# nianticlabs/wavelet-monodepth

Measured on AMD Instinct MI355X. Metric: decoder+IDWT frames/sec @640x192 bs12, higher is better.
Workload: dtype f32; 1 GPU; KITTI ResNet18 640x192 dense wavelet decoder + 4x Haar IDWT, forward, batch 12 per GPU (BASELINE.json configs[1]); encoder features resident in HBM; batch_per_gpu=12, global_batch=12, parallelism=dp1 (independent shards)

## Files before the change

wavelet_monodepth_amd/csrc/wmd_conv_fwd.hip:

```cpp
#include <algorithm>
#include <cstdlib>
#include <cstring>
#include <type_traits>
#include "wmd_conv_common.h"

namespace wmd {

template <int TH, int TW, int MR, int NR, int WM, int WN, int CK, int TAPS, int NBUF = 2>
struct ConvTile {
    static constexpr int NT = WM * WN * 64;
    static constexpr int HALO = (TAPS == 9) ? 1 : 0;
    static constexpr int PH = TH + 2 * HALO;
    static constexpr int PW = TW + 2 * HALO;
    static constexpr int NPOSITIONS = PH * PW;
    static constexpr int PS = ((NPOSITIONS - 16 + 31) / 32) * 32 + 16;
    static constexpr int NPOS = (NPOSITIONS + NT - 1) / NT;
    static constexpr int NPIX = TH * TW;
    static constexpr int A_RUN = (CK / 4) * TAPS * 64;
    static constexpr int A_FLOATS = WM * MR * A_RUN;
    static constexpr int B_FLOATS = CK * PS;
    static constexpr int NAV = (A_FLOATS / 4 + NT - 1) / NT;
    static constexpr int LDS_FLOATS = NBUF * (B_FLOATS + A_FLOATS);
    static_assert(WN * NR * 16 >= NPIX, "tile has more pixels than MFMA columns");
    static_assert(CK % 4 == 0, "CK must be a whole number of 4-channel K-steps");
    static_assert(A_FLOATS % 4 == 0, "the weight tile is moved in 16-byte pieces (a partial last wave is exec-masked)");
    static_assert(TW % 4 == 0, "four consecutive pixels of an accumulator row must not straddle image rows");
};

template <int TH, int TW, int MR, int NR, int WM, int WN, int CK, int TAPS, bool FUSE = false, int NBUF = 2>
__global__ __launch_bounds__(WM* WN * 64) void conv_fwd_kernel(const ConvKArgs a) {
    using T = ConvTile<TH, TW, MR, NR, WM, WN, CK, TAPS, NBUF>;
    constexpr int NT = T::NT, HALO = T::HALO, PW = T::PW, PS = T::PS, NPOS = T::NPOS;
    constexpr int KSTEPS = CK / 4;

    constexpr int MID_FLOATS = FUSE ? WM * MR * 16 * T::PS : 0;
    __shared__ __attribute__((aligned(16))) float lds[T::LDS_FLOATS > MID_FLOATS ? T::LDS_FLOATS : MID_FLOATS];
    float* ldsA = lds + NBUF * T::B_FLOATS;
    const int tid = threadIdx.x;
    const int lane = tid & 63;
    const int wave = __builtin_amdgcn_readfirstlane(tid >> 6);
    const int wm = wave % WM;
    const int wn = wave / WM;

    int t, by;
    if (a.cob > 0) {
        const int item = xcd_contiguous(blockIdx.x, gridDim.x);
        t = item / a.cob;
        by = item - t * a.cob;
    } else {
        t = xcd_contiguous(blockIdx.x, gridDim.x);
        by = blockIdx.y;
    }
    const int tx = t % a.tiles_x;
    t /= a.tiles_x;
    const int ty = t % a.tiles_y;
    const int b = t / a.tiles_y;
    const int y0 = ty * TH, x0 = tx * TW;
    const int ks = blockIdx.z;
    const int H = a.H, W = a.W;

    constexpr unsigned kOOB = 0x80000000u;
    unsigned ob1[NPOS], ob2[NPOS];
#pragma unroll
    for (int i = 0; i < NPOS; ++i) {
        const int p = tid + i * NT;
        const int py = p / PW, px = p % PW;
        int gy = y0 + py - HALO, gx = x0 + px - HALO;
        bool ok = p < T::NPOSITIONS;
        if (HALO) {
            ok = pad_coord(gy, H, a.pad_mode) && ok;
            ok = pad_coord(gx, W, a.pad_mode) && ok;
        }
        ok = ok && gy < H && gx < W && gy >= 0 && gx >= 0;
        gy = min(max(gy, 0), H - 1);
        gx = min(max(gx, 0), W - 1);
        ob2[i] = ok ? (unsigned)(gy * W + gx) * 4u : kOOB;
        int sy = gy - a.shift1, sx = gx - a.shift1;
        if (a.up1 == 2) {
            sy = gy >> 1;
            sx = gx >> 1;
        }
        const bool ok1 = ok && sy >= 0 && sx >= 0 && sy < a.H1 && sx < a.W1;
        ob1[i] = ok1 ? (unsigned)(sy * a.W1 + sx) * 4u : kOOB;
    }

    const size_t plane1 = (size_t)a.H1 * a.W1, plane2 = (size_t)H * W;
    const float* x1b = a.x1 + (size_t)b * a.C1 * plane1;
// ... 80 lines not shown
#pragma unroll
            for (int m = 0; m < MR; ++m) wf[slot][m] = asrc[m * T::A_RUN + (kk * TAPS + tp) * 64];
#pragma unroll
            for (int n = 0; n < NR; ++n) pf[slot][n] = bsrc[boff[n] + kk * 4 * PS + ky * PW + kx];
        };
#pragma unroll
        for (int s = 0; s < D && s < S; ++s) fetch(s);
#pragma unroll
        for (int s = 0; s < S; ++s) {
            if constexpr (PREFETCH) {
#pragma unroll
                for (int q = 0; q < NPIECES; ++q)
                    if (q * SP / NPIECES == s) stage_piece(c + 1, buf ^ 1, q);
            }
            if (s + D < S) fetch(s + D);
            __builtin_amdgcn_sched_barrier(0);
#pragma unroll
            for (int m = 0; m < MR; ++m)
#pragma unroll
                for (int n = 0; n < NR; ++n)
                    acc[m][n] = __builtin_amdgcn_mfma_f32_16x16x4f32(pf[s % RS][n], wf[s % RS][m], acc[m][n], 0, 0, 0);
            __builtin_amdgcn_sched_barrier(0);
        }
        __syncthreads();
    };
    if constexpr (NBUF == 2) {
        for (int c = c_begin; c + 1 < c_end; ++c) chunk_body(c, std::true_type{});
        if (c_begin < c_end) chunk_body(c_end - 1, std::false_type{});
    } else {
        for (int c = c_begin; c < c_end; ++c) chunk_body(c, std::false_type{});
    }

    if constexpr (FUSE) {
        static_assert(!FUSE || TAPS == 1, "the fused head is a 1x1 chain");
        constexpr int CO_T = WM * MR * 16, PS2 = T::PS, R2W = WM >= 2 ? 1 : 2;
        float* mid = lds;
#pragma unroll
        for (int m = 0; m < MR; ++m) {
            const int chl = (wm * MR + m) * 16 + (lane & 15);
            const float bv = bias_v[m];
#pragma unroll
            for (int n = 0; n < NR; ++n) {
                const int q = (wn * NR + n) * 16 + (lane >> 4) * 4;
                float4 v;
                v.x = act_apply(acc[m][n][0] + bv, a.act, a.slope);
                v.y = act_apply(acc[m][n][1] + bv, a.act, a.slope);
                v.z = act_apply(acc[m][n][2] + bv, a.act, a.slope);
                v.w = act_apply(acc[m][n][3] + bv, a.act, a.slope);
                *reinterpret_cast<float4*>(mid + chl * PS2 + q) = v;
            }
        }
        __syncthreads();
        if (WM > 2 && wm >= 2) return;
        f32x4 acc2[R2W][NR];
#pragma unroll
        for (int j = 0; j < R2W; ++j)
#pragma unroll
            for (int n = 0; n < NR; ++n) acc2[j][n] = f32x4{0.f, 0.f, 0.f, 0.f};
        constexpr int NCI4_2 = CO_T / 4;
        const float* w2 = a.wp2 + (size_t)by * (2 * NCI4_2 * 64) + lane;
        const float* msrc = mid + (lane >> 4) * PS2 + (lane & 15);
        constexpr int QD = NCI4_2 < 8 ? NCI4_2 : 8;
        float wq[QD][R2W];
#pragma unroll
        for (int q = 0; q < QD; ++q)
#pragma unroll
            for (int j = 0; j < R2W; ++j) wq[q][j] = w2[((WM == 1 ? j : wm) * NCI4_2 + q) * 64];
#pragma unroll
        for (int k4 = 0; k4 < NCI4_2; ++k4) {
            float pf[NR], wf[R2W];
#pragma unroll
            for (int j = 0; j < R2W; ++j) wf[j] = wq[k4 % QD][j];
            if (k4 + QD < NCI4_2) {
#pragma unroll
                for (int j = 0; j < R2W; ++j) wq[k4 % QD][j] = w2[((WM == 1 ? j : wm) * NCI4_2 + k4 + QD) * 64];
            }
#pragma unroll
            for (int n = 0; n < NR; ++n) pf[n] = msrc[k4 * 4 * PS2 + (wn * NR + n) * 16];
#pragma unroll
            for (int j = 0; j < R2W; ++j)
#pragma unroll
                for (int n = 0; n < NR; ++n) acc2[j][n] = __builtin_amdgcn_mfma_f32_16x16x4f32(pf[n], wf[j], acc2[j][n], 0, 0, 0);
        }
        const bool vec = (W & 3) == 0;
#pragma unroll
        for (int j = 0; j < R2W; ++j) {
            const int r2 = (WM == 1 ? j : wm) * 16 + (lane & 15);
            if (r2 >= 27) continue;
            float* tb = a.t + ((size_t)b * a.t_ctot + a.t_row0 + by * 27 + r2) * plane2;
#pragma unroll
            for (int n = 0; n < NR; ++n) {
                const int ox = x0 + (wn * NR + n) * 16 + (lane >> 4) * 4;
                if (ox >= W) continue;
                if (vec && ox + 3 < W) {
                    *reinterpret_cast<float4*>(tb + ox) = make_float4(acc2[j][n][0], acc2[j][n][1], acc2[j][n][2], acc2[j][n][3]);
                } else {
#pragma unroll
                    for (int r = 0; r < 4; ++r)
                        if (ox + r < W) tb[ox + r] = acc2[j][n][r];
                }
            }
        }
        return;
    }

    const bool final_out = (a.ksplit == 1);
    float* ybase = a.y + ((size_t)ks * a.B + b) * a.Cout * plane2;
    const bool vec_ok = (W & 3) == 0;
#pragma unroll
    for (int m = 0; m < MR; ++m) {
        const int co = ((by * WM + wm) * MR + m) * 16 + (lane & 15);
        const float bv = final_out ? bias_v[m] : 0.f;
#pragma unroll
        for (int n = 0; n < NR; ++n) {
            const int q = (wn * NR + n) * 16 + (lane >> 4) * 4;
            const int oy = y0 + q / TW, ox = x0 + q % TW;
            if (co >= a.Cout || q >= T::NPIX || oy >= H || ox >= W) continue;
            float v[4];
#pragma unroll
            for (int r = 0; r < 4; ++r) {
                v[r] = acc[m][n][r];
                if (final_out) v[r] = act_apply(v[r] + bv, a.act, a.slope);
            }
            float* dst = ybase + (size_t)co * plane2 + (size_t)oy * W + ox;
            if (final_out && a.gate) {
                const float* gp = a.gate + ((size_t)b * a.Cout + co) * plane2 + (size_t)oy * W + ox;
                if (vec_ok && ox + 3 < W) {
                    const float4 gv = *reinterpret_cast<const float4*>(gp);
                    v[0] *= act_deriv(gv.x, a.gate_act, a.gate_slope);
                    v[1] *= act_deriv(gv.y, a.gate_act, a.gate_slope);
                    v[2] *= act_deriv(gv.z, a.gate_act, a.gate_slope);
                    v[3] *= act_deriv(gv.w, a.gate_act, a.gate_slope);
                } else {
#pragma unroll
                    for (int r = 0; r < 4; ++r)
                        if (ox + r < W) v[r] *= act_deriv(gp[r], a.gate_act, a.gate_slope);
                }
            }
            if (vec_ok && ox + 3 < W) {
                *reinterpret_cast<float4*>(dst) = make_float4(v[0], v[1], v[2], v[3]);
            } else {
#pragma unroll
                for (int r = 0; r < 4; ++r)
                    if (ox + r < W) dst[r] = v[r];
            }
        }
    }
}

__global__ void conv_splitk_reduce_kernel(const float* __restrict__ partial, const float* __restrict__ bias,
                                          float* __restrict__ y, size_t n, size_t plane, int Cout, int ksplit,
                                          int act, float slope, const float* __restrict__ gate, int gate_act, float gate_slope,
                                          const uint8_t* __restrict__ out_mask) {
    for (size_t i = (size_t)blockIdx.x * blockDim.x + threadIdx.x; i < n; i += (size_t)gridDim.x * blockDim.x) {
        float v = 0.f;
        int s = 0;
        if (out_mask && out_mask[i / (plane * Cout) * plane + i % plane] == 0) {
            y[i] = 0.f;
            continue;
        }
        for (; s + 4 <= ksplit; s += 4) {
            const float p0 = partial[(size_t)s * n + i], p1 = partial[(size_t)(s + 1) * n + i];
            const float p2 = partial[(size_t)(s + 2) * n + i], p3 = partial[(size_t)(s + 3) * n + i];
            v = (((v + p0) + p1) + p2) + p3;
        }
        for (; s < ksplit; ++s) v += partial[(size_t)s * n + i];
        if (bias) v += bias[(i / plane) % Cout];
        v = act_apply(v, act, slope);
        if (gate) v *= act_deriv(gate[i], gate_act, gate_slope);
        y[i] = v;
    }
}

constexpr int kRedCh = 8;
__global__ __launch_bounds__(256) void conv_splitk_reduce_list_kernel(const float* __restrict__ partial, const float* __restrict__ bias,
                                                                      float* __restrict__ y, const int* __restrict__ tile_list,
                                                                      const int* __restrict__ tile_count, const uint8_t* __restrict__ out_mask,
                                                                      int B, int Cout, int H, int W, int TH, int TW, int tiles_x, int tiles_y,
                                                                      int cob, int nchunks, int ksmax, int slots, int act, float slope) {
    const int n_act = list_total(tile_count, B);
    if ((int)blockIdx.x >= n_act) return;
    int ks, cps;
    list_ksplit(n_act * cob, nchunks, ksmax, slots, ks, cps);
// ... 1075 lines not shown
```

wavelet_monodepth_amd/csrc/wmd_head.hip:

```cpp
#include <algorithm>
#include <cstdlib>
#include "wmd_internal.h"
#include "wmd_head_shiftsum.h"

namespace wmd {



constexpr int HT_H = 16, HT_W = 32, H_CK = 8, H_TT = 128;
constexpr int H_PH = HT_H + 2;
constexpr int H_PWV = HT_W + 2;
constexpr int H_PW = 36;
constexpr int H_PS = H_PH * H_PW + 4;

template <int COUT>
struct HeadSmem {
    float patch[2][H_CK * H_PS];
    float wgt[2][H_CK * COUT * 12];
    float dump[64];
};

template <int COUT, int NG>
__device__ __forceinline__ void head_side(const float* __restrict__ x, size_t bstride, const float* __restrict__ wgt,
                                          int C, int c_begin, int c_end, int H, int W, int b, int y0, int x0,
// ... 188 lines not shown
                sp[q] = 1.f / (1.f + expf(-accp[co][q]));
                if (a.mode == 1) {
                    r[q] = a.scale * sp[q];
                } else {
                    sn[q] = 1.f / (1.f + expf(-accn[co][q]));
                    r[q] = a.scale * sp[q] - a.scale * sn[q];
                }
            }
        }
        float* yo = a.y + o + co * plane;
        if (vec) {
            *reinterpret_cast<float4*>(yo) = make_float4(r[0], r[1], r[2], r[3]);
            if (a.mode >= 1 && a.sig_p) *reinterpret_cast<float4*>(a.sig_p + o + co * plane) = make_float4(sp[0], sp[1], sp[2], sp[3]);
            if (a.mode == 2 && a.sig_n) *reinterpret_cast<float4*>(a.sig_n + o + co * plane) = make_float4(sn[0], sn[1], sn[2], sn[3]);
        } else {
#pragma unroll
            for (int q = 0; q < 4; ++q)
                if (ox + q < a.W) {
                    yo[q] = r[q];
                    if (a.mode >= 1 && a.sig_p) a.sig_p[o + co * plane + q] = sp[q];
                    if (a.mode == 2 && a.sig_n) a.sig_n[o + co * plane + q] = sn[q];
                }
        }
    }
}

__global__ void head_finalize_kernel(const wmd_head_args a, const float* __restrict__ partial, int csplit) {
    const size_t plane = (size_t)a.H * a.W;
    const size_t n = (size_t)a.B * a.Cout * plane;
    for (size_t i = (size_t)blockIdx.x * blockDim.x + threadIdx.x; i < n; i += (size_t)gridDim.x * blockDim.x) {
        const size_t pix = i % plane;
        const int co = (i / plane) % a.Cout;
        const int b = i / (plane * a.Cout);
        float p = a.bias_p ? a.bias_p[co] : 0.f, q = (a.mode == 2 && a.bias_n) ? a.bias_n[co] : 0.f;
        for (int cs = 0; cs < csplit; ++cs) {
            const float* pp = partial + (((size_t)cs * a.B + b) * 2 * a.Cout) * plane + pix;
            p += pp[(size_t)co * plane];
            if (a.mode == 2) q += pp[(size_t)(a.Cout + co) * plane];
        }
        float r;
        if (a.mode == 0) {
            r = a.scale * p;
        } else {
            const float sp = 1.f / (1.f + expf(-p));
            if (a.sig_p) a.sig_p[i] = sp;
            if (a.mode == 1) {
                r = a.scale * sp;
            } else {
                const float sn = 1.f / (1.f + expf(-q));
                if (a.sig_n) a.sig_n[i] = sn;
                r = a.scale * sp - a.scale * sn;
            }
        }
        a.y[i] = r;
    }
}

__global__ void head_shiftsum_kernel(const wmd_head_shiftsum_args a) {
    const int H = a.H, W = a.W;
    const size_t plane = (size_t)H * W;
    const size_t total = (size_t)a.B * plane;
    const size_t total_w = (total + 63) / 64 * 64;
    for (size_t i0 = (size_t)blockIdx.x * blockDim.x + threadIdx.x; i0 < total_w; i0 += (size_t)gridDim.x * blockDim.x) {
        const bool live = i0 < total;
        const size_t i = live ? i0 : total - 1;
        const int x = i % W;
        const int y = (i / W) % H;
        const size_t b = i / plane;
        int off[9];
        float okf[9];
#pragma unroll
        for (int t = 0; t < 9; ++t) {
            int gy = y + t / 3 - 1, gx = x + t % 3 - 1;
            const bool ok = pad_coord(gy, H, a.pad_mode) & pad_coord(gx, W, a.pad_mode);
            gy = min(max(gy, 0), H - 1);
            gx = min(max(gx, 0), W - 1);
            off[t] = gy * W + gx;
            okf[t] = ok ? 1.f : 0.f;
        }
        const float* tb = a.t + b * (a.yl_out ? 81 : 54) * plane;
        const bool in_mask = !a.yh_mask || a.yh_mask[b * plane + (size_t)y * W + x] != 0;
        const bool wave_any = __builtin_amdgcn_ballot_w64(in_mask && live) != 0;
        float yh[3] = {0.f, 0.f, 0.f};
        if (wave_any) {
            float vp[27], vn[27];
#pragma unroll
            for (int k = 0; k < 27; ++k) {
                vp[k] = tb[(size_t)k * plane + off[k % 9]];
                vn[k] = tb[(size_t)(27 + k) * plane + off[k % 9]];
            }
#pragma unroll
            for (int co = 0; co < 3; ++co) {
                float sp = a.bias_p ? a.bias_p[co] : 0.f, sn = a.bias_n ? a.bias_n[co] : 0.f;
#pragma unroll
                for (int t = 0; t < 9; ++t) {
                    sp += okf[t] * vp[co * 9 + t];
                    sn += okf[t] * vn[co * 9 + t];
                }
                const float a1 = fast_sigmoid(sp), a2 = fast_sigmoid(sn);
                yh[co] = in_mask ? a.scale * a1 - a.scale * a2 : 0.f;
                if (a.sig_p && live) {
                    a.sig_p[(b * 3 + co) * plane + (size_t)y * W + x] = a1;
                    a.sig_n[(b * 3 + co) * plane + (size_t)y * W + x] = a2;
                }
            }
        }
        if (live) {
#pragma unroll
            for (int co = 0; co < 3; ++co) a.yh[(b * 3 + co) * plane + (size_t)y * W + x] = yh[co];
        }
        float l = 0.f;
        if (a.yl_out) {
            float sl = a.bias_ll ? a.bias_ll[0] : 0.f;
#pragma unroll
            for (int t = 0; t < 9; ++t) sl += okf[t] * tb[(size_t)(54 + t) * plane + off[t]];
            const float sgl = fast_sigmoid(sl);
            l = a.scale_ll * sgl;
            if (live) a.yl_out[i] = l;
            if (live && a.sig_ll) a.sig_ll[i] = sgl;
        } else if (a.yl) {
            l = a.yl[i];
        }
        if ((a.yl || a.yl_out) && a.out) {
            float v[4] = {(l + yh[0] + yh[1] + yh[2]) * 0.5f, (l + yh[0] - yh[1] - yh[2]) * 0.5f,
                          (l - yh[0] + yh[1] - yh[2]) * 0.5f, (l - yh[0] - yh[1] + yh[2]) * 0.5f};
            if (a.range_keys) {
                float lo = live ? fminf(fminf(v[0], v[1]), fminf(v[2], v[3])) : INFINITY;
                float hi = live ? fmaxf(fmaxf(v[0], v[1]), fmaxf(v[2], v[3])) : -INFINITY;
                const int b0 = __builtin_amdgcn_readfirstlane((int)b);
                const bool uniform = __builtin_amdgcn_ballot_w64((int)b != b0) == 0;
                if (uniform) {
#pragma unroll
                    for (int o = 32; o > 0; o >>= 1) {
                        lo = fminf(lo, __shfl_xor(lo, o));
                        hi = fmaxf(hi, __shfl_xor(hi, o));
                    }
                }
                if ((uniform ? (threadIdx.x & 63) == 0 : live) && lo <= hi) {
                    const unsigned ul = __float_as_uint(lo), uh = __float_as_uint(hi);
                    atomicMin(&a.range_keys[2 * b], (ul & 0x80000000u) ? ~ul : (ul | 0x80000000u));
                    atomicMax(&a.range_keys[2 * b + 1], (uh & 0x80000000u) ? ~uh : (uh | 0x80000000u));
                }
            }
            if (!live) continue;
            const size_t dst = b * 4 * plane + (size_t)(2 * y) * (2 * W) + 2 * x;
            *reinterpret_cast<float2*>(a.out + dst) = make_float2(v[0], v[1]);
            *reinterpret_cast<float2*>(a.out + dst + 2 * W) = make_float2(v[2], v[3]);
            if (a.disp) {
#pragma unroll
                for (int k = 0; k < 4; ++k) {
                    v[k] *= a.disp_scale;
                    if (a.clamp01) v[k] = fminf(fmaxf(v[k], 0.f), 1.f);
                }
                *reinterpret_cast<float2*>(a.disp + dst) = make_float2(v[0], v[1]);
                *reinterpret_cast<float2*>(a.disp + dst + 2 * W) = make_float2(v[2], v[3]);
            }
        }
    }
}

struct ShiftsumChainArgs {
    wmd_head_shiftsum_args lv[3];
    int n;
    int by0, bx0;
};


__global__ __launch_bounds__(256) void head_shiftsum_chain_kernel(const ShiftsumChainArgs c) {
    __shared__ float low[2][256];
    const int by0 = c.by0, bx0 = c.bx0;
    const int H0 = c.lv[0].H, W0 = c.lv[0].W;
    const int tiles_x = (W0 + bx0 - 1) / bx0, tiles_y = (H0 + by0 - 1) / by0;
    int t = blockIdx.x;
    const int tx = t % tiles_x;
    t /= tiles_x;
    const int ty = t % tiles_y;
    const size_t b = t / tiles_y;
    const int tid = threadIdx.x;
    for (int k = 0; k < c.n; ++k) {
        const int sy = by0 << k, sx = bx0 << k;
        if (tid < sy * sx) {
            const int py = tid / sx, px = tid % sx;
            const int y = ty * sy + py, x = tx * sx + px;
            if (y < c.lv[k].H && x < c.lv[k].W) {
                float v[4];
                shiftsum_pixel(c.lv[k], b, y, x, k > 0, k > 0 ? low[(k - 1) & 1][py * sx + px] : 0.f, v);
                if (k + 1 < c.n) {
                    float* nl = low[k & 1];
                    const int ns = sx * 2;
                    nl[(2 * py) * ns + 2 * px] = v[0];
                    nl[(2 * py) * ns + 2 * px + 1] = v[1];
                    nl[(2 * py + 1) * ns + 2 * px] = v[2];
                    nl[(2 * py + 1) * ns + 2 * px + 1] = v[3];
                }
            }
        }
        __syncthreads();
    }
// ... 122 lines not shown
```

wavelet_monodepth_amd/csrc/wmd_head_chain.hip:

```cpp
#include <algorithm>
#include <cstdlib>
#include <type_traits>
#include <utility>
#include "wmd_internal.h"

#ifndef WMD_CHAIN_PD256
#define WMD_CHAIN_PD256 4
#endif
#ifndef WMD_CHAIN_PD128
#define WMD_CHAIN_PD128 1
#endif

namespace wmd {

typedef float f32x4 __attribute__((ext_vector_type(4)));

template <class F, int... I>
__device__ __forceinline__ void hc_static_for_impl(F&& f, std::integer_sequence<int, I...>) {
    (f(std::integral_constant<int, I>{}), ...);
}
template <int N, class F>
__device__ __forceinline__ void hc_static_for(F&& f) {
    hc_static_for_impl(f, std::make_integer_sequence<int, N>{});
}

__device__ __forceinline__ void hc_barrier() {
    asm volatile("s_waitcnt lgkmcnt(0)" ::: "memory");
    __builtin_amdgcn_s_barrier();
    asm volatile("" ::: "memory");
}

struct HeadChainArgs {
    const float* x;
    const float* wp1;
    const float* bias1;
    const float* wp2;
    float* t;
    int plane, tiles, t_planes;
    int C;
    float slope;
    const uint8_t* run_mask;
    const float* ll_wp1;
    const float* ll_bias1;
    const float* ll_wp2;
    float* mid_out;
    int mid_ct, mid_off[3];
};

template <int C, int RS, int PG, int NT, int KC>
struct HeadChainTile {
    static constexpr int NW = RS * PG, NTH = NW * 64;
    static constexpr int PXB = PG * NT * 16;
    static constexpr int MTS = C / 16;
    static constexpr int MT = MTS / RS;
    static constexpr int KS = C / 4;
    static constexpr int NCH = KS / KC;
    static constexpr int XS = PXB % 32 == 0 ? PXB + 16 : PXB + 32;
    static constexpr int WF = MTS * KC * 64;
    static constexpr int XF = KC * 4 * XS;
    static constexpr int NBUF = NCH > 1 ? 2 : 1;
    static constexpr int WV = (WF / 4 + NTH - 1) / NTH;
    static constexpr int XV = (KC * PXB + NTH - 1) / NTH;
    static constexpr int RED = RS > 1 ? NW * 3 * NT * 256 : 0;
    static constexpr int WFL = (C == 256 && RS == 4) ? RS * KC * 64 : 0;
    static constexpr int STAGE = NBUF * (WF + WFL + XF);
    static constexpr int LDS_FLOATS = STAGE > RED ? STAGE : RED;
    static_assert(C % 16 == 0 && MTS % RS == 0 && KS % KC == 0, "whole tiles");
    static_assert(XS % 32 == 16 && PXB % 4 == 0, "bank-conflict-free x rows");
};

template <class T, int KC, bool LLX>
__device__ __forceinline__ void chain_fetch(f32x4 (&wreg)[T::WV], f32x4 (&xreg)[T::XV], f32x4& lreg, const float* __restrict__ w1,
                                            const float* __restrict__ wl, const float* __restrict__ xb, int c, int tid, int pix0, int plane) {
    if constexpr (LLX) {
        static_assert(T::WFL > 0 && T::WFL / 4 <= T::NTH, "one 16-byte piece per thread covers the low-pass part of a chunk");
        const int f = tid * 4, m = f / (KC * 64), rem = f % (KC * 64);
        if (f < T::WFL) lreg = *reinterpret_cast<const f32x4*>(wl + ((size_t)m * T::KS + c * KC) * 64 + rem);
    }
#pragma unroll
    for (int v = 0; v < T::WV; ++v) {
        const int f = (v * T::NTH + tid) * 4;
        const int m = f / (KC * 64), rem = f % (KC * 64);
        f32x4 wv = {0.f, 0.f, 0.f, 0.f};
        if (T::WF % (4 * T::NTH) == 0 || f < T::WF) wv = *reinterpret_cast<const f32x4*>(w1 + ((size_t)m * T::KS + c * KC) * 64 + rem);
        wreg[v] = wv;
    }
#pragma unroll
    for (int v = 0; v < T::XV; ++v) {
        const int q = v * T::NTH + tid;
        const int chl = q / (T::PXB / 4), px = pix0 + (q % (T::PXB / 4)) * 4;
        f32x4 val = {0.f, 0.f, 0.f, 0.f};
        if (q < KC * T::PXB && px < plane)
            val = *reinterpret_cast<const f32x4*>(xb + (size_t)(c * KC * 4 + chl) * plane + px);
        xreg[v] = val;
    }
}

template <class T, int KC, bool LLX>
__device__ __forceinline__ void chain_commit(const f32x4 (&wreg)[T::WV], const f32x4 (&xreg)[T::XV], const f32x4& lreg, float* ws, int tid) {
    float* xs = ws + T::WF + T::WFL;
    if constexpr (LLX) {
        if (tid * 4 < T::WFL) *reinterpret_cast<f32x4*>(ws + T::WF + tid * 4) = lreg;
    }
#pragma unroll
    for (int v = 0; v < T::WV; ++v)
        if (T::WF % (4 * T::NTH) == 0 || (v * T::NTH + tid) * 4 < T::WF) *reinterpret_cast<f32x4*>(ws + (v * T::NTH + tid) * 4) = wreg[v];
#pragma unroll
    for (int v = 0; v < T::XV; ++v) {
        const int q = v * T::NTH + tid;
        if (q < KC * T::PXB) *reinterpret_cast<f32x4*>(xs + (q / (T::PXB / 4)) * T::XS + (q % (T::PXB / 4)) * 4) = xreg[v];
    }
}

template <int C, int RS, int PG, int NT, int KC, bool LLX, int PD>
__device__ __forceinline__ void head_chain_body(const HeadChainArgs& a, float* lds, const int bx, const int side) {
    using T = HeadChainTile<C, RS, PG, NT, KC>;
    constexpr int MT = T::MT, KS = T::KS, XS = T::XS, PXB = T::PXB;
    constexpr int MTX = MT + (LLX ? 1 : 0);
    static_assert(!LLX || (C / 4) / 16 == RS, "the low-pass chain: C/4 mid channels = one row tile per channel slice");

    const int tid = threadIdx.x, lane = tid & 63;
    const int wave = __builtin_amdgcn_readfirstlane(tid >> 6);
    const int r = wave % RS, pg = wave / RS;
    const int g = lane >> 4, lc = lane & 15;
    const int tile = bx % a.tiles, b = bx / a.tiles;
    const int pix0 = tile * PXB, plane = a.plane;
    if (a.run_mask) {
        static_assert(PXB <= T::NTH, "one mask byte per thread covers the block's pixel run");
        __shared__ int run_any[T::NW];
        const bool mine = tid < PXB && pix0 + tid < plane && a.run_mask[(size_t)b * plane + pix0 + tid] != 0;
        const bool wave_any = __builtin_amdgcn_ballot_w64(mine) != 0;
        if (lane == 0) run_any[wave] = wave_any ? 1 : 0;
        __syncthreads();
        int all = 0;
#pragma unroll
        for (int w = 0; w < T::NW; ++w) all |= run_any[w];
        if (all == 0) return;
    }
    const float* xb = a.x + (size_t)b * C * plane;
    const float* w1 = a.wp1 + (size_t)side * T::MTS * KS * 64;
    const float* w2 = a.wp2 + (size_t)side * 2 * KS * 64;

    static_assert(PD >= 1 && (T::NCH % PD == 0 || T::NCH == 1), "the chunk loop is unrolled by the prefetch distance");
    f32x4 wreg[PD][T::WV], xreg[PD][T::XV], lreg[PD];
#pragma unroll
    for (int d = 0; d < PD; ++d) lreg[d] = f32x4{0.f, 0.f, 0.f, 0.f};
    constexpr int BUF = T::WF + T::WFL + T::XF;

    f32x4 acc[MTX][NT];
#pragma unroll
    for (int m = 0; m < MTX; ++m)
#pragma unroll
        for (int n = 0; n < NT; ++n) acc[m][n] = f32x4{0.f, 0.f, 0.f, 0.f};

    chain_fetch<T, KC, LLX>(wreg[0], xreg[0], lreg[0], w1, a.ll_wp1, xb, 0, tid, pix0, plane);
    chain_commit<T, KC, LLX>(wreg[0], xreg[0], lreg[0], lds, tid);
    hc_static_for<PD>([&](auto kc) __attribute__((always_inline)) {
        constexpr int k = decltype(kc)::value + 1;
        if (k < T::NCH) chain_fetch<T, KC, LLX>(wreg[k % PD], xreg[k % PD], lreg[k % PD], w1, a.ll_wp1, xb, k, tid, pix0, plane);
    });
    hc_barrier();
    for (int c0 = 0; c0 < T::NCH; c0 += PD) {
        hc_static_for<PD>([&](auto dc) __attribute__((always_inline)) {
            constexpr int d = decltype(dc)::value, dn = (d + 1) % PD;
            const int c = c0 + d;
            const float* ws = lds + (c & (T::NBUF - 1)) * BUF;
            const float* xs = ws + T::WF + T::WFL;
#pragma unroll
            for (int kk = 0; kk < KC; ++kk) {
                float xf[NT], wf[MTX];
#pragma unroll
                for (int n = 0; n < NT; ++n) xf[n] = xs[(kk * 4 + g) * XS + (pg * NT + n) * 16 + lc];
#pragma unroll
                for (int m = 0; m < MT; ++m) wf[m] = ws[((r * MT + m) * KC + kk) * 64 + lane];
                if constexpr (LLX) wf[MT] = ws[T::WF + (r * KC + kk) * 64 + lane];
#pragma unroll
                for (int m = 0; m < MTX; ++m)
#pragma unroll
                    for (int n = 0; n < NT; ++n) acc[m][n] = __builtin_amdgcn_mfma_f32_16x16x4f32(wf[m], xf[n], acc[m][n], 0, 0, 0);
            }
            if (c + 1 < T::NCH) {
                chain_commit<T, KC, LLX>(wreg[dn], xreg[dn], lreg[dn], lds + ((c + 1) & (T::NBUF - 1)) * BUF, tid);
                if (c + 1 + PD < T::NCH)
                    chain_fetch<T, KC, LLX>(wreg[dn], xreg[dn], lreg[dn], w1, a.ll_wp1, xb, c + 1 + PD, tid, pix0, plane);
                hc_barrier();
            }
        });
    }

    f32x4 acc2[2][NT];
#pragma unroll
    for (int j = 0; j < 2; ++j)
#pragma unroll
        for (int n = 0; n < NT; ++n) acc2[j][n] = f32x4{0.f, 0.f, 0.f, 0.f};
#pragma unroll
    for (int m = 0; m < MT; ++m) {
        const int mg = r * MT + m;
        float bv[4] = {0.f, 0.f, 0.f, 0.f};
        if (a.bias1) {
            const float4 b4 = *reinterpret_cast<const float4*>(a.bias1 + side * C + mg * 16 + g * 4);
            bv[0] = b4.x, bv[1] = b4.y, bv[2] = b4.z, bv[3] = b4.w;
        }
        float w2f[2][4];
#pragma unroll
        for (int j = 0; j < 2; ++j)
#pragma unroll
            for (int i = 0; i < 4; ++i) w2f[j][i] = w2[((size_t)j * KS + 4 * mg + g) * 64 + i * 16 + lc];
#pragma unroll
        for (int i = 0; i < 4; ++i) {
#pragma unroll
            for (int n = 0; n < NT; ++n) {
                const float mid = act_apply(acc[m][n][i] + bv[i], WMD_ACT_LEAKY, a.slope);
                if (a.mid_out) {
                    const int px = pix0 + (pg * NT + n) * 16 + lc;
                    if (px < plane) a.mid_out[((size_t)b * a.mid_ct + a.mid_off[side] + mg * 16 + g * 4 + i) * plane + px] = mid;
                }
#pragma unroll
                for (int j = 0; j < 2; ++j) acc2[j][n] = __builtin_amdgcn_mfma_f32_16x16x4f32(w2f[j][i], mid, acc2[j][n], 0, 0, 0);
            }
        }
    }

    f32x4 acc2l[NT];
#pragma unroll
    for (int n = 0; n < NT; ++n) acc2l[n] = f32x4{0.f, 0.f, 0.f, 0.f};
    if constexpr (LLX) {
        float bv[4] = {0.f, 0.f, 0.f, 0.f};
        if (a.ll_bias1) {
            const float4 b4 = *reinterpret_cast<const float4*>(a.ll_bias1 + r * 16 + g * 4);
            bv[0] = b4.x, bv[1] = b4.y, bv[2] = b4.z, bv[3] = b4.w;
        }
        float w2l[4];
#pragma unroll
        for (int i = 0; i < 4; ++i) w2l[i] = a.ll_wp2[((size_t)4 * r + g) * 64 + i * 16 + lc];
#pragma unroll
        for (int i = 0; i < 4; ++i)
#pragma unroll
            for (int n = 0; n < NT; ++n) {
                const float mid = act_apply(acc[MT][n][i] + bv[i], WMD_ACT_LEAKY, a.slope);
                if (a.mid_out) {
                    const int px = pix0 + (pg * NT + n) * 16 + lc;
                    if (px < plane) a.mid_out[((size_t)b * a.mid_ct + a.mid_off[2] + r * 16 + g * 4 + i) * plane + px] = mid;
                }
                acc2l[n] = __builtin_amdgcn_mfma_f32_16x16x4f32(w2l[i], mid, acc2l[n], 0, 0, 0);
            }
    }

    if constexpr (RS > 1) {
        constexpr int NJ = LLX ? 3 : 2;
        __syncthreads();
        float* red = lds + (size_t)wave * 3 * NT * 256;
#pragma unroll
        for (int j = 0; j < NJ; ++j)
#pragma unroll
            for (int n = 0; n < NT; ++n) {
                const f32x4 v = j < 2 ? acc2[j < 2 ? j : 0][n] : acc2l[n];
                *reinterpret_cast<float4*>(red + ((j * NT + n) * 64 + lane) * 4) = make_float4(v[0], v[1], v[2], v[3]);
            }
        __syncthreads();
        if (r != 0) return;
#pragma unroll
        for (int j = 0; j < NJ; ++j)
#pragma unroll
            for (int n = 0; n < NT; ++n) {
                float4 s = *reinterpret_cast<const float4*>(lds + (size_t)(pg * RS) * 3 * NT * 256 + ((j * NT + n) * 64 + lane) * 4);
#pragma unroll
                for (int rr = 1; rr < RS; ++rr) {
                    const float4 p = *reinterpret_cast<const float4*>(lds + (size_t)(pg * RS + rr) * 3 * NT * 256 + ((j * NT + n) * 64 + lane) * 4);
                    s.x += p.x, s.y += p.y, s.z += p.z, s.w += p.w;
                }
                if (j < 2) acc2[j < 2 ? j : 0][n] = f32x4{s.x, s.y, s.z, s.w};
                else acc2l[n] = f32x4{s.x, s.y, s.z, s.w};
            }
    }

    float* tb = a.t + ((size_t)b * a.t_planes + side * 27) * plane;
#pragma unroll
    for (int n = 0; n < NT; ++n) {
        const int px = pix0 + (pg * NT + n) * 16 + lc;
        if (px >= plane) continue;
#pragma unroll
        for (int j = 0; j < 2; ++j)
#pragma unroll
            for (int i = 0; i < 4; ++i) {
                const int row = j * 16 + g * 4 + i;
                if (row < 27) tb[(size_t)row * plane + px] = acc2[j][n][i];
            }
        if constexpr (LLX) {
#pragma unroll
            for (int i = 0; i < 4; ++i) {
                const int row = g * 4 + i;
                if (row < 9) tb[(size_t)(54 + row) * plane + px] = acc2l[n][i];
            }
        }
    }
}

template <int C, int RS, int PG, int NT, int KC, int PD, bool LLC = false>
__global__ __launch_bounds__(RS* PG * 64, (RS * PG >= 8 ? 3 : 1)) void head_chain_kernel(const HeadChainArgs a) {
    using T = HeadChainTile<C, RS, PG, NT, KC>;
    __shared__ __attribute__((aligned(16))) float lds[T::LDS_FLOATS];
    if constexpr (LLC) {
        if (blockIdx.y == 0) {
            head_chain_body<C, RS, PG, NT, KC, true, PD>(a, lds, blockIdx.x, 0);
            return;
        }
    }
    head_chain_body<C, RS, PG, NT, KC, false, PD>(a, lds, blockIdx.x, blockIdx.y);
}

struct HeadChainMulti {
    HeadChainArgs lv[3];
    int first[4];
    int n;
};
constexpr int head_chain_multi_lds() {
    int m = HeadChainTile<256, 4, 1, 1, 4>::LDS_FLOATS;
    if (HeadChainTile<128, 1, 4, 1, 8>::LDS_FLOATS > m) m = HeadChainTile<128, 1, 4, 1, 8>::LDS_FLOATS;
    if (HeadChainTile<64, 1, 4, 2, 16>::LDS_FLOATS > m) m = HeadChainTile<64, 1, 4, 2, 16>::LDS_FLOATS;
    return m;
}
__global__ __launch_bounds__(256, 3) void head_chain_multi_kernel(const HeadChainMulti m) {
    __shared__ __attribute__((aligned(16))) float lds[head_chain_multi_lds()];
    int k = 0;
    while (k + 1 < m.n && (int)blockIdx.x >= m.first[k + 1]) ++k;
    const HeadChainArgs& a = m.lv[k];
    const int v = (int)blockIdx.x - m.first[k], per_side = (m.first[k + 1] - m.first[k]) >> 1;
    const int side = v >= per_side ? 1 : 0, bx = v - side * per_side;
    if (a.C == 256) {
        if (side == 0 && a.ll_wp1) head_chain_body<256, 4, 1, 1, 4, true, WMD_CHAIN_PD256>(a, lds, bx, 0);
        else head_chain_body<256, 4, 1, 1, 4, false, WMD_CHAIN_PD256>(a, lds, bx, side);
    } else if (a.C == 128) {
        head_chain_body<128, 1, 4, 1, 8, false, WMD_CHAIN_PD128>(a, lds, bx, side);
    } else {
        head_chain_body<64, 1, 4, 2, 16, false, 1>(a, lds, bx, side);
    }
}

template <int C, int RS, int PG, int NT, int KC, int PD>
static void launch_chain(const HeadChainArgs& a, int B, hipStream_t s) {
    using T = HeadChainTile<C, RS, PG, NT, KC>;
    HeadChainArgs k = a;
    k.tiles = (a.plane + T::PXB - 1) / T::PXB;
    if constexpr (C == 256 && RS == 4) {
        if (a.ll_wp1) {
            hipLaunchKernelGGL((head_chain_kernel<C, RS, PG, NT, KC, PD, true>), dim3((unsigned)(B * k.tiles), 2), dim3(T::NTH), 0, s, k);
            return;
        }
    }
    hipLaunchKernelGGL((head_chain_kernel<C, RS, PG, NT, KC, PD>), dim3((unsigned)(B * k.tiles), 2), dim3(T::NTH), 0, s, k);
}

static HeadChainArgs head_chain_args(const wmd_head_fused_args* g, int t_planes, long plane, bool& with_ll) {
    HeadChainArgs a;
    a.x = g->x;
    a.wp1 = g->wp1;
    a.bias1 = g->bias1;
    a.wp2 = g->wp2;
    a.t = g->t;
    a.plane = (int)plane;
    a.tiles = 0;
    a.t_planes = t_planes;
    a.slope = g->slope;
    a.run_mask = g->run_mask;
    with_ll = g->ll_wp1 && g->ll_wp2 && g->C == 256 && t_planes == 81 && !g->run_mask;
    a.ll_wp1 = with_ll ? g->ll_wp1 : nullptr;
    a.ll_bias1 = with_ll ? g->ll_bias1 : nullptr;
    a.ll_wp2 = with_ll ? g->ll_wp2 : nullptr;
    a.mid_out = g->mid_out;
    a.mid_ct = g->mid_ct;
    a.mid_off[0] = g->mid_off_p;
    a.mid_off[1] = g->mid_off_n;
    a.mid_off[2] = g->mid_off_ll;
    a.C = g->C;
    return a;
}

int head_chain_launch(const wmd_head_fused_args* g, int t_planes, hipStream_t s) {
    static const bool on = [] {
        const char* e = getenv("WMD_HEAD_CHAIN");
        return !(e && atoi(e) == 0);
    }();
    const long plane = (long)g->H * g->W;
    if (!on || (plane & 3) || plane > (1L << 28) || (g->C != 64 && g->C != 128 && g->C != 256)) return 0;
    bool with_ll = false;
    HeadChainArgs a = head_chain_args(g, t_planes, plane, with_ll);
    const double pix = (double)g->B * plane;
    ProfScope prof("head_chain_kernel", 2.0 * pix * (2.0 * g->C * g->C + 54.0 * g->C), 4.0 * pix * (g->C + 54), s);
    if (g->C == 64)
        launch_chain<64, 1, 4, 2, 16, 1>(a, g->B, s);
    else if (g->C == 128)
        launch_chain<128, 1, 4, 1, 8, WMD_CHAIN_PD128>(a, g->B, s);
    else {
        static const int pg_force = [] {
            const char* e = getenv("WMD_HEAD_CHAIN_PG256");
            return e ? atoi(e) : 0;
        }();
        const long b32 = (long)g->B * ((plane + 31) / 32) * 2, b48 = (long)g->B * ((plane + 47) / 48) * 2;
        const long cost32 = ((b32 + kNumCU - 1) / kNumCU) * 2, cost48 = ((b48 + kNumCU - 1) / kNumCU) * 3;
        if (pg_force == 3 || (pg_force == 0 && cost48 < cost32)) launch_chain<256, 4, 3, 1, 4, WMD_CHAIN_PD256>(a, g->B, s);
        else launch_chain<256, 4, 2, 1, 4, WMD_CHAIN_PD256>(a, g->B, s);
    }
    return with_ll ? 2 : 1;
}

int head_chain_multi_launch(const wmd_head_fused_args* g, int n, hipStream_t s) {
    static const bool on = [] {
        const char* e = getenv("WMD_HEAD_CHAIN_MULTI");
        const char* c = getenv("WMD_HEAD_CHAIN");
        return !(e && atoi(e) == 0) && !(c && atoi(c) == 0);
    }();
// ... 29 lines not shown
```

wavelet_monodepth_amd/csrc/wmd_head_shiftsum.h:

```cpp
#pragma once
#include "wmd_internal.h"

namespace wmd {

__device__ __forceinline__ float fast_sigmoid(float h) { return __builtin_amdgcn_rcpf(1.f + __expf(-h)); }

__device__ __forceinline__ bool shiftsum_gather(const wmd_head_shiftsum_args& a, size_t b, int y, int x, float (&yh)[3], float& l) {
    const int H = a.H, W = a.W;
    const size_t plane = (size_t)H * W, i = b * plane + (size_t)y * W + x;
    int off[9];
    float okf[9];
#pragma unroll
    for (int t = 0; t < 9; ++t) {
        int gy = y + t / 3 - 1, gx = x + t % 3 - 1;
        const bool ok = pad_coord(gy, H, a.pad_mode) & pad_coord(gx, W, a.pad_mode);
        gy = min(max(gy, 0), H - 1);
        gx = min(max(gx, 0), W - 1);
        off[t] = gy * W + gx;
        okf[t] = ok ? 1.f : 0.f;
    }
    const float* tb = a.t + b * (a.yl_out ? 81 : 54) * plane;
    float vp[27], vn[27];
#pragma unroll
    for (int k = 0; k < 27; ++k) {
        vp[k] = tb[(size_t)k * plane + off[k % 9]];
        vn[k] = tb[(size_t)(27 + k) * plane + off[k % 9]];
    }
#pragma unroll
    for (int co = 0; co < 3; ++co) {
        float sp = a.bias_p ? a.bias_p[co] : 0.f, sn = a.bias_n ? a.bias_n[co] : 0.f;
#pragma unroll
        for (int t = 0; t < 9; ++t) {
            sp += okf[t] * vp[co * 9 + t];
            sn += okf[t] * vn[co * 9 + t];
        }
        const float a1 = fast_sigmoid(sp), a2 = fast_sigmoid(sn);
        yh[co] = a.scale * a1 - a.scale * a2;
        a.yh[(b * 3 + co) * plane + (size_t)y * W + x] = yh[co];
    }
    if (a.yl_out) {
        float sl = a.bias_ll ? a.bias_ll[0] : 0.f;
#pragma unroll
        for (int t = 0; t < 9; ++t) sl += okf[t] * tb[(size_t)(54 + t) * plane + off[t]];
        l = a.scale_ll * fast_sigmoid(sl);
        a.yl_out[i] = l;
        return true;
    }
    if (a.yl) {
        l = a.yl[i];
        return true;
    }
    return false;
}

__device__ __forceinline__ void shiftsum_finish(const wmd_head_shiftsum_args& a, size_t b, int y, int x, const float (&yh)[3], float l, float (&v)[4]) {
    const int W = a.W;
    const size_t plane = (size_t)a.H * W;
    v[0] = (l + yh[0] + yh[1] + yh[2]) * 0.5f;
    v[1] = (l + yh[0] - yh[1] - yh[2]) * 0.5f;
    v[2] = (l - yh[0] + yh[1] - yh[2]) * 0.5f;
    v[3] = (l - yh[0] - yh[1] + yh[2]) * 0.5f;
    if (a.out) {
        const size_t dst = b * 4 * plane + (size_t)(2 * y) * (2 * W) + 2 * x;
        *reinterpret_cast<float2*>(a.out + dst) = make_float2(v[0], v[1]);
        *reinterpret_cast<float2*>(a.out + dst + 2 * W) = make_float2(v[2], v[3]);
        if (a.disp) {
            float d[4];
#pragma unroll
            for (int k = 0; k < 4; ++k) {
                d[k] = v[k] * a.disp_scale;
                if (a.clamp01) d[k] = fminf(fmaxf(d[k], 0.f), 1.f);
            }
            *reinterpret_cast<float2*>(a.disp + dst) = make_float2(d[0], d[1]);
            *reinterpret_cast<float2*>(a.disp + dst + 2 * W) = make_float2(d[2], d[3]);
        }
    }
}

__device__ __forceinline__ void shiftsum_pixel(const wmd_head_shiftsum_args& a, size_t b, int y, int x, bool have_l_in, float l_in, float (&v)[4]) {
    float yh[3], l = 0.f;
    const bool own = shiftsum_gather(a, b, y, x, yh, l);
    if (!own) l = have_l_in ? l_in : 0.f;
    shiftsum_finish(a, b, y, x, yh, l, v);
}

}
```

Before: 23710 frames/s.

## Store head tap planes pixel-major in per-tap groups for vectorised shiftsum gathers

Changes the intermediate tap tensor from planar channel-major layout to a pixel-major layout where each pixel's 9 taps store their 6 or 7 values (three positive, three negative, optional low-pass) contiguously. Producers (conv epilogue and head chain) write grouped values and the weight rows are permuted to match. The shiftsum consumers can then load each tap with a vector load instead of 54-63 scattered scalar loads. The head-chain block-to-side mapping is also interleaved in groups of 8 so the two sides are processed together. The risk is that producer stores become strided and less coalesced.

```diff
diff --git a/wavelet_monodepth_amd/csrc/wmd_conv_fwd.hip b/wavelet_monodepth_amd/csrc/wmd_conv_fwd.hip
--- a/wavelet_monodepth_amd/csrc/wmd_conv_fwd.hip
+++ b/wavelet_monodepth_amd/csrc/wmd_conv_fwd.hip
@@ -3,6 +3,7 @@
 #include <cstring>
 #include <type_traits>
 #include "wmd_conv_common.h"
+#include "wmd_head_taps.h"
 
 namespace wmd {
 
@@ -249,23 +250,20 @@
 #pragma unroll
                 for (int n = 0; n < NR; ++n) acc2[j][n] = __builtin_amdgcn_mfma_f32_16x16x4f32(pf[n], wf[j], acc2[j][n], 0, 0, 0);
         }
-        const bool vec = (W & 3) == 0;
+        const int G = tap_group_floats(a.t_ctot);
+        const bool ll = a.t_row0 != 0;
 #pragma unroll
         for (int j = 0; j < R2W; ++j) {
             const int r2 = (WM == 1 ? j : wm) * 16 + (lane & 15);
-            if (r2 >= 27) continue;
-            float* tb = a.t + ((size_t)b * a.t_ctot + a.t_row0 + by * 27 + r2) * plane2;
+            if (r2 >= (ll ? 9 : 27)) continue;
+            const int tap = r2 % 9, slot = ll ? TAP_SLOT_LL : (int)by * TAP_SLOT_N + r2 / 9;
+            float* tb = a.t + (size_t)b * a.t_ctot * plane2 + slot;
 #pragma unroll
             for (int n = 0; n < NR; ++n) {
                 const int ox = x0 + (wn * NR + n) * 16 + (lane >> 4) * 4;
-                if (ox >= W) continue;
-                if (vec && ox + 3 < W) {
-                    *reinterpret_cast<float4*>(tb + ox) = make_float4(acc2[j][n][0], acc2[j][n][1], acc2[j][n][2], acc2[j][n][3]);
-                } else {
-#pragma unroll
-                    for (int r = 0; r < 4; ++r)
-                        if (ox + r < W) tb[ox + r] = acc2[j][n][r];
-                }
+#pragma unroll
+                for (int r = 0; r < 4; ++r)
+                    if (ox + r < W) tb[tap_group_index(ox + r, tap, G)] = acc2[j][n][r];
             }
         }
         return;
diff --git a/wavelet_monodepth_amd/csrc/wmd_head.hip b/wavelet_monodepth_amd/csrc/wmd_head.hip
--- a/wavelet_monodepth_amd/csrc/wmd_head.hip
+++ b/wavelet_monodepth_amd/csrc/wmd_head.hip
@@ -294,13 +294,15 @@
         const bool in_mask = !a.yh_mask || a.yh_mask[b * plane + (size_t)y * W + x] != 0;
         const bool wave_any = __builtin_amdgcn_ballot_w64(in_mask && live) != 0;
         float yh[3] = {0.f, 0.f, 0.f};
+        float vl[9];
+        if (a.yl_out && !wave_any) {
+#pragma unroll
+            for (int t = 0; t < 9; ++t) vl[t] = tb[tap_group_index((size_t)off[t], t, 7) + TAP_SLOT_LL];
+        }
         if (wave_any) {
             float vp[27], vn[27];
-#pragma unroll
-            for (int k = 0; k < 27; ++k) {
-                vp[k] = tb[(size_t)k * plane + off[k % 9]];
-                vn[k] = tb[(size_t)(27 + k) * plane + off[k % 9]];
-            }
+            if (a.yl_out) shiftsum_taps<7>(tb, off, vp, vn, vl);
+            else shiftsum_taps<6>(tb, off, vp, vn, vl);
 #pragma unroll
             for (int co = 0; co < 3; ++co) {
                 float sp = a.bias_p ? a.bias_p[co] : 0.f, sn = a.bias_n ? a.bias_n[co] : 0.f;
@@ -325,7 +327,7 @@
         if (a.yl_out) {
             float sl = a.bias_ll ? a.bias_ll[0] : 0.f;
 #pragma unroll
-            for (int t = 0; t < 9; ++t) sl += okf[t] * tb[(size_t)(54 + t) * plane + off[t]];
+            for (int t = 0; t < 9; ++t) sl += okf[t] * vl[t];
             const float sgl = fast_sigmoid(sl);
             l = a.scale_ll * sgl;
             if (live) a.yl_out[i] = l;
diff --git a/wavelet_monodepth_amd/csrc/wmd_head_chain.hip b/wavelet_monodepth_amd/csrc/wmd_head_chain.hip
--- a/wavelet_monodepth_amd/csrc/wmd_head_chain.hip
+++ b/wavelet_monodepth_amd/csrc/wmd_head_chain.hip
@@ -2,6 +2,7 @@
 #include <cstdlib>
 #include <type_traits>
 #include <utility>
+#include "wmd_head_taps.h"
 #include "wmd_internal.h"
 
 #ifndef WMD_CHAIN_PD256
@@ -140,6 +141,12 @@
     const float* xb = a.x + (size_t)b * C * plane;
     const float* w1 = a.wp1 + (size_t)side * T::MTS * KS * 64;
     const float* w2 = a.wp2 + (size_t)side * 2 * KS * 64;
+    int w2row[2];
+#pragma unroll
+    for (int j = 0; j < 2; ++j) {
+        const int src = tap_row_source(16 * j + lc);
+        w2row[j] = (src >> 4) * KS * 64 + (src & 15);
+    }
 
     static_assert(PD >= 1 && (T::NCH % PD == 0 || T::NCH == 1), "the chunk loop is unrolled by the prefetch distance");
     f32x4 wreg[PD][T::WV], xreg[PD][T::XV], lreg[PD];
@@ -205,7 +212,7 @@
 #pragma unroll
         for (int j = 0; j < 2; ++j)
 #pragma unroll
-            for (int i = 0; i < 4; ++i) w2f[j][i] = w2[((size_t)j * KS + 4 * mg + g) * 64 + i * 16 + lc];
+            for (int i = 0; i < 4; ++i) w2f[j][i] = w2[w2row[j] + (4 * mg + g) * 64 + i * 16];
 #pragma unroll
         for (int i = 0; i < 4; ++i) {
 #pragma unroll
@@ -274,23 +281,24 @@
             }
     }
 
-    float* tb = a.t + ((size_t)b * a.t_planes + side * 27) * plane;
+    struct __attribute__((packed, aligned(4))) f3 { float x, y, z; };
+    const int G = tap_group_floats(a.t_planes);
+    float* tb = a.t + (size_t)b * a.t_planes * plane + side * TAP_SLOT_N;
 #pragma unroll
     for (int n = 0; n < NT; ++n) {
         const int px = pix0 + (pg * NT + n) * 16 + lc;
         if (px >= plane) continue;
 #pragma unroll
-        for (int j = 0; j < 2; ++j)
+        for (int j = 0; j < 2; ++j) {
+            const int e = 2 * g + j;
+            *reinterpret_cast<f3*>(tb + tap_group_index(px, e, G)) = f3{acc2[j][n][0], acc2[j][n][1], acc2[j][n][2]};
+            if (e < 3) tb[tap_group_index(px, 8, G) + e] = acc2[j][n][3];
+        }
+        if constexpr (LLX) {
 #pragma unroll
             for (int i = 0; i < 4; ++i) {
-                const int row = j * 16 + g * 4 + i;
-                if (row < 27) tb[(size_t)row * plane + px] = acc2[j][n][i];
-            }
-        if constexpr (LLX) {
-#pragma unroll
-            for (int i = 0; i < 4; ++i) {
-                const int row = g * 4 + i;
-                if (row < 9) tb[(size_t)(54 + row) * plane + px] = acc2l[n][i];
+                const int tap = g * 4 + i;
+                if (tap < 9) tb[tap_group_index(px, tap, G) + TAP_SLOT_LL] = acc2l[n][i];
             }
         }
     }
@@ -326,7 +334,15 @@
     while (k + 1 < m.n && (int)blockIdx.x >= m.first[k + 1]) ++k;
     const HeadChainArgs& a = m.lv[k];
     const int v = (int)blockIdx.x - m.first[k], per_side = (m.first[k + 1] - m.first[k]) >> 1;
-    const int side = v >= per_side ? 1 : 0, bx = v - side * per_side;
+    const int full = per_side & ~7, tail = per_side - full;
+    int side, bx;
+    if (v < 2 * full) {
+        side = (v >> 3) & 1;
+        bx = (v >> 4) * 8 + (v & 7);
+    } else {
+        side = v - 2 * full >= tail ? 1 : 0;
+        bx = full + (v - 2 * full) - side * tail;
+    }
     if (a.C == 256) {
         if (side == 0 && a.ll_wp1) head_chain_body<256, 4, 1, 1, 4, true, WMD_CHAIN_PD256>(a, lds, bx, 0);
         else head_chain_body<256, 4, 1, 1, 4, false, WMD_CHAIN_PD256>(a, lds, bx, side);
diff --git a/wavelet_monodepth_amd/csrc/wmd_head_shiftsum.h b/wavelet_monodepth_amd/csrc/wmd_head_shiftsum.h
--- a/wavelet_monodepth_amd/csrc/wmd_head_shiftsum.h
+++ b/wavelet_monodepth_amd/csrc/wmd_head_shiftsum.h
@@ -1,7 +1,34 @@
 #pragma once
+#include "wmd_head_taps.h"
 #include "wmd_internal.h"
 
 namespace wmd {
+
+template <int G>
+__device__ __forceinline__ void shiftsum_taps(const float* tb, const int (&off)[9], float (&vp)[27], float (&vn)[27], float (&vl)[9]) {
+    typedef float v4 __attribute__((ext_vector_type(4)));
+    typedef float v2 __attribute__((ext_vector_type(2)));
+    typedef v4 v4_a8 __attribute__((aligned(8)));
+    typedef v4 v4_a4 __attribute__((aligned(4)));
+    typedef v2 v2_g __attribute__((aligned(8)));
+    struct __attribute__((packed, aligned(4))) s3 { float x, y, z; };
+    static_assert(G == 6 || G == 7, "three + values, three - values (and the low-pass one)");
+#pragma unroll
+    for (int t = 0; t < 9; ++t) {
+        const float* p = tb + tap_group_index((size_t)off[t], t, G);
+        v4 lo;
+        if constexpr (G == 6) lo = *reinterpret_cast<const v4_a8*>(p);
+        else lo = *reinterpret_cast<const v4_a4*>(p);
+        vp[t] = lo[0], vp[9 + t] = lo[1], vp[18 + t] = lo[2], vn[t] = lo[3];
+        if constexpr (G == 6) {
+            const v2 hi = *reinterpret_cast<const v2_g*>(p + 4);
+            vn[9 + t] = hi[0], vn[18 + t] = hi[1];
+        } else {
+            const s3 hi = *reinterpret_cast<const s3*>(p + 4);
+            vn[9 + t] = hi.x, vn[18 + t] = hi.y, vl[t] = hi.z;
+        }
+    }
+}
 
 __device__ __forceinline__ float fast_sigmoid(float h) { return __builtin_amdgcn_rcpf(1.f + __expf(-h)); }
 
@@ -20,12 +47,9 @@
         okf[t] = ok ? 1.f : 0.f;
     }
     const float* tb = a.t + b * (a.yl_out ? 81 : 54) * plane;
-    float vp[27], vn[27];
-#pragma unroll
-    for (int k = 0; k < 27; ++k) {
-        vp[k] = tb[(size_t)k * plane + off[k % 9]];
-        vn[k] = tb[(size_t)(27 + k) * plane + off[k % 9]];
-    }
+    float vp[27], vn[27], vl[9];
+    if (a.yl_out) shiftsum_taps<7>(tb, off, vp, vn, vl);
+    else shiftsum_taps<6>(tb, off, vp, vn, vl);
 #pragma unroll
     for (int co = 0; co < 3; ++co) {
         float sp = a.bias_p ? a.bias_p[co] : 0.f, sn = a.bias_n ? a.bias_n[co] : 0.f;
@@ -41,7 +65,7 @@
     if (a.yl_out) {
         float sl = a.bias_ll ? a.bias_ll[0] : 0.f;
 #pragma unroll
-        for (int t = 0; t < 9; ++t) sl += okf[t] * tb[(size_t)(54 + t) * plane + off[t]];
+        for (int t = 0; t < 9; ++t) sl += okf[t] * vl[t];
         l = a.scale_ll * fast_sigmoid(sl);
         a.yl_out[i] = l;
         return true;
diff --git a/wavelet_monodepth_amd/csrc/wmd_head_taps.h b/wavelet_monodepth_amd/csrc/wmd_head_taps.h
--- /dev/null
+++ b/wavelet_monodepth_amd/csrc/wmd_head_taps.h
@@ -0,0 +1,17 @@
+#pragma once
+#include <stddef.h>
+
+namespace wmd {
+
+constexpr int TAP_SLOT_N = 3;
+constexpr int TAP_SLOT_LL = 6;
+
+__host__ __device__ constexpr int tap_group_floats(int t_planes) { return t_planes == 81 ? 7 : 6; }
+__host__ __device__ constexpr size_t tap_group_index(size_t pixel, int tap, int G) { return (pixel * 9 + (size_t)tap) * (size_t)G; }
+
+__host__ __device__ constexpr int tap_row_source(int R) {
+    const int j = R >> 4, g = (R >> 2) & 3, i = R & 3, e = 2 * g + j;
+    return i < 3 ? i * 9 + e : (e < 3 ? e * 9 + 8 : 31);
+}
+
+}
```

After: 23820 frames/s (median of 6 runs). Within noise of the previous version (+0.4%).
